# cgrigis/drynx

Hardware: AMD Instinct MI355X
Metric: end-to-end query latency + range-proof verifications/sec, logreg on 1e6 records (higher is better)
Workload: dtype bn254-exact/fp64

## Files before the change

csrc/kernels/dx_gt_t2.hip:

```cpp
#define DX_NI __host__ __device__ __forceinline__
#include "common.h"

namespace {
constexpr int kChunk = 8;

DX_HD bool fp_canonical(const uint32_t *w) {
  uint32_t br = 0;
  for (int k = 0; k < 8; k++) (void)subb32(w[k], FpParams::MOD[k], br);
  return br != 0;
}

DX_HD void compress_chunk(const uint32_t *a, uint32_t *c, uint8_t *ok, int64_t i0, int64_t i1) {
  Fp6 acc = Fp6::one();
  uint32_t good = 0;
  for (int64_t i = i0; i < i1; i++) {
    const uint32_t *w = a + 96 * i;
    bool g = true;
    for (int k = 0; k < 12; k++) g = g && fp_canonical(w + 8 * k);
    const Fp12 f = at<Fp12>(a, i);
    g = g && !(f.c1 == Fp6::zero()) && sub(sqr(f.c0), mul_v(sqr(f.c1))) == Fp6::one();
    at<Fp6>(c, i) = acc;
    if (g) {
      good |= 1u << (i - i0);
      acc = mul(acc, f.c1);
// ... 114 lines not shown
  if (!on_gpu) return kChunk;
  const int64_t c = n / (1024 * 64 * 2);
  return c < 1 ? 1 : (c > kChunk ? kChunk : c);
}

int dx_gt_t2_compress(int on_gpu, void *stream, const uint32_t *a, uint32_t *c, uint8_t *ok, int64_t n) {
  const int64_t k = t2_chunk(on_gpu, n);
  const int64_t chunks = (n + k - 1) / k;
  auto op = [=] __host__ __device__(int64_t t) {
    const int64_t i0 = t * k, i1 = i0 + k < n ? i0 + k : n;
    compress_chunk(a, c, ok, i0, i1);
  };
  return run(on_gpu, stream, chunks, op, true, "gt_t2_compress");
}

int dx_gt_t2_decompress(int on_gpu, void *stream, const uint32_t *c, uint32_t *a, int64_t n) {
  const int64_t k = t2_chunk(on_gpu, n);
  const int64_t chunks = (n + k - 1) / k;
  auto op = [=] __host__ __device__(int64_t t) {
    const int64_t i0 = t * k, i1 = i0 + k < n ? i0 + k : n;
    decompress_chunk(c, a, i0, i1);
  };
  return run(on_gpu, stream, chunks, op, true, "gt_t2_decompress");
}
}
```

csrc/kernels/dx_range.hip:

```cpp
#include "common.h"
#include "../bn254/gt_coop.h"

extern "C" {

int dx_rp_prove_a(int on_gpu, void *stream, const uint32_t *negsB_aff, const uint32_t *V_aff, const uint32_t *t_sc,
                  const uint32_t *gt_table, uint32_t *a_out, int64_t n_items, int S, int L) {
  auto op = [=] __host__ __device__(int64_t it) {
    int64_t j = it % L;
    int64_t p = it / ((int64_t)S * L);
    int64_t pj = p * L + j;
    Fp12 f = final_exp(miller_loop(at<G1A>(negsB_aff, pj), at<G2A>(V_aff, it)));
    Fp12 g = gt_fixed_pow(reinterpret_cast<const Fp12 *>(gt_table), t_sc + 8 * pj);
    at<Fp12>(a_out, it) = mul(f, g);
  };
  return run(on_gpu, stream, n_items, op, true, "rp_prove_a");
}

int dx_rp_prove_a_tab(int on_gpu, void *stream, const uint32_t *gphi_tables, const int32_t *tab_idx,
                      const uint32_t *e_sc, const uint32_t *t_sc, const uint32_t *gt_table, uint32_t *a_out,
                      int64_t n_items, int S, int L, int wbits) {
  const int64_t n_pj = n_items / S;
  auto p1 = [=] __host__ __device__(int64_t pj) {
    const int64_t p = pj / L, j = pj % L;
    at<Fp12>(a_out, p * S * L + j) = gt_fixed_pow(reinterpret_cast<const Fp12 *>(gt_table), t_sc + 8 * pj);
// ... 41 lines not shown
  if (n_slices <= 0) return 0;
  if (!on_gpu) {
    host_for_each(n_slices, [=](int64_t s) {
      const int64_t b = start[s];
      const int n = len[s];
      Fp12 acc = Fp12::one();
      for (int k = 0; k < n; k++) acc = mul(acc, at<Fp12>(src, idx ? idx[b + k] : b + k));
      at<Fp12>(out, s) = acc;
    });
    return 0;
  }
  const unsigned blocks = (unsigned)((n_slices + coop::kTriples - 1) / coop::kTriples);
  hipLaunchKernelGGL(gt_slice_prod_coop, dim3(blocks), dim3(64), 0, (hipStream_t)stream, src, idx, start, len, out,
                     n_slices);
  return check_hip(hipGetLastError(), "gt_slice_prod");
}

namespace {
__global__ void __launch_bounds__(64) DX_OCC gt_chunk_weight_coop(const uint32_t *B, const int32_t *d,
                                                                 const int64_t *start, const int32_t *len,
                                                                 const int32_t *base, uint32_t *out,
                                                                 int64_t n_chunks) {
  const coop::Role R = coop::role();
  const int64_t ch = (int64_t)blockIdx.x * coop::kTriples + R.g;
  if (R.g >= coop::kTriples || ch >= n_chunks) return;
  const Fp12 *F = reinterpret_cast<const Fp12 *>(B);
  const int64_t a = start[ch];
  const int n = len[ch];
  const uint32_t b0 = (uint32_t)base[ch];
  Fp6 acc = coop::one(R), tot = coop::one(R);
// ... 55 lines not shown
```

drynx_amd/native/__init__.py:

```python
from __future__ import annotations

import ctypes
import os
import threading

import numpy as np

import torch

_HERE = os.path.dirname(os.path.abspath(__file__))
LIB_PATH = os.environ.get("DRYNX_NATIVE_LIB") or os.path.join(_HERE, "libdrynx_native.so")

_lib = None


def _load():
    global _lib
    if _lib is not None:
        return _lib
    if not os.path.exists(LIB_PATH):
        if os.environ.get("DRYNX_AUTOBUILD", "1") == "1":
            from . import build as _b

            _b.build()
# ... 107 lines not shown
    "dx_g2_joint_table": [_I, _P, _P, _P, _L],
    "dx_g2_joint_table_signed": [_I, _P, _P, _P, _P, _L],
    "dx_rp_u_group": [_I, _P, _P, _P, _P, _P, _P, _P, _L, _I, _L, _I, _I, _L, _P, _P],
    "dx_rp_u_joint": [_I, _P, _P, _P, _P, _L, _I, _I, _L, _P],
    "dx_g2_slice_sum": [_I, _P, _P, _P, _P, _P, _P, _L, _I, _L],
    "dx_g2_horner": [_I, _P, _P, _P, _I, _I, _I, _L, _L],
    "dx_rp_msm_uv": [_I, _P, _P, _P, _L, _I, _L],
    "dx_msm_keys": [_I, _P, _P, _P, _L, _L, _I, _I, _P, _P],
    "dx_gls8_entries": [],
    "dx_g2_gls8_table": [_I, _P, _P, _P, _P, _L],
    "dx_gt_gls8_table": [_I, _P, _P, _P, _P, _L, _P, _L],
    "dx_g2_gls8_mul": [_I, _P, _P, _P, _P, _P, _L],
    "dx_rp_prove_a_gls8": [_I, _P, _P, _P, _P, _P, _P, _P, _L, _I, _I, _I, _P],
    "dx_gt16_entries": [],
    "dx_gt16_table": [_I, _P, _P, _P, _P],
}


def _declare(lib):
    for name, args in _SIGS.items():
        fn = getattr(lib, name)
        fn.argtypes = args
        fn.restype = ctypes.c_int


def lib():
    return _load()


def loaded_path() -> str:
# ... 145 lines not shown
    _call("dx_g1_fb_mul_i64", g, s, _ptr(table), _ptr(m.contiguous()), _ptr(out), n)
    return out


G1_MUL_PAIR_ROWS = 1 << 14


def gt_t2_compress(a: torch.Tensor, out: torch.Tensor | None = None):
    n = _rows(a, 96)
    c = torch.empty((n, 48), dtype=torch.int32, device=a.device) if out is None else out
    assert c.is_contiguous() and _rows(c, 48) == n
    ok = torch.empty((n,), dtype=torch.uint8, device=a.device)
    g, s = _ctx(a, c)
    _call("dx_gt_t2_compress", g, s, _ptr(a.contiguous()), _ptr(c), _ptr(ok), n)
    return ok if out is not None else (c, ok)


def gt_t2_decompress(c: torch.Tensor, out: torch.Tensor | None = None) -> torch.Tensor:
    n = _rows(c, 48)
    out = torch.empty((n, 96), dtype=torch.int32, device=c.device) if out is None else out
    assert out.is_contiguous() and _rows(out, 96) == n
    g, s = _ctx(c, out)
    _call("dx_gt_t2_decompress", g, s, _ptr(c.contiguous()), _ptr(out), n)
    return out


def g2_x_compress(V: torch.Tensor, x_out: torch.Tensor | None = None, flag_out: torch.Tensor | None = None):
    n = _rows(V, 32)
    x = torch.empty((n, 16), dtype=torch.int32, device=V.device) if x_out is None else x_out
    f = torch.empty((n,), dtype=torch.int32, device=V.device) if flag_out is None else flag_out
# ... 1105 lines not shown
        cur = _gt_prod_level(cur, 8)
    return gt_prod(cur.cpu(), chunk=4).view(1, 96)


def _gt_prod_level(x: torch.Tensor, ch: int) -> torch.Tensor:
    n_items, n_groups = x.shape[0], x.shape[1]
    n_chunks = (n_items + ch - 1) // ch
    out = torch.empty((n_chunks, n_groups, 96), dtype=torch.int32, device=x.device)
    g, s = _ctx(x)
    _call("dx_gt_prod_chunks", g, s, _ptr(x.contiguous()), _ptr(out), n_items, n_groups, ch)
    return out


from .msm import (G2_CHUNK, capture_keep, check_overflow, g1_msm, g1_msm_device, g1_msm_finish,
                  g1_msm_grouped, g1_msm_launch, g1_msm_plan, g1_slice_sum, g2_chunk_weight, g2_msm_device,
                  g2_msm_finish, g2_msm_launch, g2_msm_run, g2_slice_sum, gt_chunk_weight, gt_slice_prod, me_window,
                  multi_exp_device, multi_exp_grouped, multi_exp_grouped_finish, multi_exp_plan, rp_msm_uv)
```

drynx_amd/native/msm.py:

```python
from __future__ import annotations

import threading

import numpy as np

import torch

from . import (_call, _ctx, _gt_prod_level, _pow2_scalar, _ptr, _raw_call, _rows, _upload, g1_mul, gt_mul, gt_one,
               gt_pow, gt_prod)

_ME_SLICE = 8
G2_CHUNK = 32


def gt_slice_prod(src: torch.Tensor, idx, start: torch.Tensor, length: torch.Tensor) -> torch.Tensor:
    n = start.numel()
    out = torch.empty((n, 96), dtype=torch.int32, device=src.device)
    g, s = _ctx(src, idx, start, length)
    _call("dx_gt_slice_prod", g, s, _ptr(src), _ptr(idx), _ptr(start), _ptr(length), _ptr(out), n)
    return out


def g1_slice_sum(src: torch.Tensor, idx, start: torch.Tensor, length: torch.Tensor) -> torch.Tensor:
    n = start.numel()
    out = torch.empty((n, 24), dtype=torch.int32, device=src.device)
    g, s = _ctx(src, idx, start, length)
    _call("dx_g1_slice_sum", g, s, _ptr(src), _ptr(idx), _ptr(start), _ptr(length), _ptr(out), n)
    return out


def g2_slice_sum(src: torch.Tensor, idx, start: torch.Tensor, length: torch.Tensor, src_aff: bool,
                 idx_mod: int = 0) -> torch.Tensor:
    n = start.numel()
    assert src.shape[-1] == (32 if src_aff else 48) and (idx is None or idx.dtype == torch.int32)
# ... 17 lines not shown

def g2_chunk_weight(B_jac: torch.Tensor, d: torch.Tensor, start: torch.Tensor, length: torch.Tensor,
                    base: torch.Tensor) -> torch.Tensor:
    n = start.numel()
    assert B_jac.shape[-1] == 48 and d.dtype == torch.int32 and start.dtype == torch.int64
    assert length.dtype == torch.int32 and base.dtype == torch.int32 and base.numel() == n
    out = torch.empty((n, 48), dtype=torch.int32, device=B_jac.device)
    g, s = _ctx(B_jac, d, start, length, base)
    _call("dx_g2_chunk_weight", g, s, _ptr(B_jac.contiguous()), _ptr(d.contiguous()), _ptr(start), _ptr(length),
          _ptr(base), _ptr(out), n)
    return out


def _gt_ops(a: torch.Tensor, items: torch.Tensor, item_split: tuple | None = None):
    n = a.shape[0]
    it = items.to(torch.int64)
    if item_split is not None:
        sp, q = item_split
        it = torch.where(it < sp, it % n, (it - sp) % q)
    else:
        it = it % n
    it = it.contiguous()
    return (lambda st, ln: gt_slice_prod(a, it, st, ln)), (lambda cur, st, ln: gt_slice_prod(cur, None, st, ln))


def _g1_ops(P_jac: torch.Tensor, items: torch.Tensor):
    P_jac, it = P_jac.contiguous(), items.to(torch.int64)
    return (lambda st, ln: g1_slice_sum(P_jac, it, st, ln)), (lambda cur, st, ln: g1_slice_sum(cur, None, st, ln))


def _g2_ops(P_aff: torch.Tensor, items: torch.Tensor, m: int):
    return (lambda st, ln: g2_slice_sum(P_aff, items, st, ln, True, m)), \
        (lambda cur, st, ln: g2_slice_sum(cur, None, st, ln, False))


def _group_arg(group, n: int, dev):
    if group is None:
        return None, 0
# ... 275 lines not shown
def multi_exp_device(a: torch.Tensor, k: torch.Tensor, group, groups: tuple, W: int | None = None,
                     c: int | None = None, item_split: tuple | None = None) -> dict:
    dev = a.device
    G = len(groups)
    if c is None:
        W, c = me_window(tuple(groups))
    B, lay, overflow = _device_buckets(k, group, groups, W, c, _ME_SLICE, lambda items: _gt_ops(a, items, item_split))
    if "gtw" not in lay:
        lay["gtw"] = _chunk_weight_plan(lay["used"], c, dev)
    wp = lay["gtw"]
    cur = gt_chunk_weight(B, wp["d"], *wp["chunks"])
    for st, ln in wp["gpasses"]:
        cur = gt_slice_prod(cur, None, st, ln)
    win = gt_one(dev).repeat(G * W, 1)
    win.index_copy_(0, wp["gws"], cur)
    return {"G": G, "W": W, "c": c, "win": win.view(1, G * W, 96), "overflow": overflow}


def multi_exp_grouped_finish(h) -> torch.Tensor:
    G, W = h["G"], h["W"]
    if h["win"] is None:
        return gt_one("cpu").repeat(G, 1)
    S_w = gt_prod(h["win"].cpu(), chunk=64).view(G, W, 96)
    acc = S_w[:, W - 1].contiguous()
    sh = _pow2_scalar(h["c"]).expand(G, 8).contiguous()
    for w in range(W - 2, -1, -1):
        acc = gt_mul(gt_pow(acc, sh), S_w[:, w].contiguous())
    return acc


# ... 111 lines not shown
```

drynx_amd/proofs/ledger_codec.py:

```python
from __future__ import annotations

import numpy as np
import torch

from .. import native as nt

MAGIC = 0x32435052
_HEAD = 5
_RW = 5
_GT, _G2 = 0, 1
_FULL = {_GT: 96, _G2: 32}
_SMALL = {_GT: 48, _G2: 17}


def _regions(b, k: int) -> np.ndarray:
    return np.frombuffer(bytes(b[4 * _HEAD: 4 * (_HEAD + _RW * k)]), dtype=np.int32).reshape(k, _RW)


def is_compressed(b) -> bool:
    if len(b) < 4 * _HEAD or len(b) % 4 or int.from_bytes(bytes(b[:4]), "little") != MAGIC:
        return False
    w = np.frombuffer(bytes(b[:4 * _HEAD]), dtype=np.int32)
    k = int(w[4])
    if int(w[1]) != 1 or k < 1 or 4 * (_HEAD + _RW * k) > len(b):
        return False
    total = int(w[2:4].view(np.int64)[0])
    r = _regions(b, k)
    if not np.isin(r[:, 4], (_GT, _G2)).all():
        return False
    m = r[:, 2:4].copy().view(np.int64).reshape(-1)
    saved = sum(int(mi) * (_FULL[int(kd)] - _SMALL[int(kd)]) for mi, kd in zip(m, r[:, 4]))
    return len(b) // 4 == _HEAD + _RW * k + total - saved


class Pending:

    def __init__(self, tensor: torch.Tensor, regions: list | None):
        self.tensor = tensor.contiguous().reshape(-1)
        self.regions = regions
        self.image = None
        self.compact = False

    def produce(self, stream):
        with torch.cuda.stream(stream):
            if self.regions is None:
                self.regions = regions_from_header(self.tensor)
            if not self.regions:
                self.compact = False
                return memoryview(self.tensor.cpu().numpy()).cast("B")
            img = self.launch()
            host = torch.empty((img.numel(),), dtype=torch.uint8, pin_memory=True)
            nt.copy_to_host([(img, host)], host)
            ev = torch.cuda.Event()
            ev.record(stream)
        ev.synchronize()
        return self.finish(memoryview(host.numpy()))

    def launch(self) -> torch.Tensor:
        t = self.tensor
        dev = t.device
        if dev.type == "cuda":
            t.record_stream(torch.cuda.current_stream(dev))
        head = [MAGIC, 0] + list(np.array([t.numel()], dtype=np.int64).view(np.int32)) + [len(self.regions)]
        for off, m, kind in self.regions:
            head += list(np.array([off, m], dtype=np.int64).view(np.int32)) + [kind]
        n_img = len(head) + t.numel() - sum(m * (_FULL[kd] - _SMALL[kd]) for _, m, kd in self.regions)
        img = torch.empty((n_img,), dtype=torch.int32, device=dev)
        hdr = torch.tensor(head, dtype=torch.int32)
        if dev.type == "cuda":
            hdr = hdr.pin_memory().to(dev, non_blocking=True)
        pairs, oks, pos, q = [(hdr, img[:len(head)])], [], 0, len(head)
        for off, m, kind in self.regions:
            pairs.append((t[pos:off], img[q: q + off - pos]))
            q += off - pos
            src = t[off: off + _FULL[kind] * m].view(m, _FULL[kind])
            if kind == _GT:
                oks.append(nt.gt_t2_compress(src, out=img[q: q + 48 * m].view(m, 48)))
            else:
                oks.append(nt.g2_x_compress(src, x_out=img[q: q + 16 * m].view(m, 16),
                                            flag_out=img[q + 16 * m: q + 17 * m])[2])
            q += _SMALL[kind] * m
            pos = off + _FULL[kind] * m
        pairs.append((t[pos:], img[q:]))
        nt.batched_copy(pairs)
        okall = torch.cat(oks).all() if len(oks) > 1 else oks[0].all()
        img[1:2].copy_(okall.to(torch.int32).view(1))
        self.image = img
        return img.view(torch.uint8)

    def finish(self, mv: memoryview):
        self.compact = int.from_bytes(bytes(mv[4:8]), "little") == 1
        if self.compact:
            return mv
        return memoryview(self.tensor.cpu().numpy()).cast("B")


def regions_from_header(t: torch.Tensor) -> list:
    W = t.numel()
    if W < 2:
        return []
    k = int(t[0])
    if k < 1 or 1 + k > W:
        return []
    lens = t[1: 1 + k].cpu().tolist()
    pos, regions = 1 + k, []
    for ln in lens:
        if ln < 5 or pos + ln > W:
            return []
        magic, n, u, l, S = t[pos: pos + 5].cpu().tolist()
# ... 74 lines not shown
```

drynx_amd/proofs/range_proof.py:

```python
from __future__ import annotations

import hashlib
import io
import math
import os
import threading
from dataclasses import dataclass

import numpy as np
import torch

from .. import native as nt
from ..crypto import bn254 as bn
from ..crypto import oracle as O
from ..crypto.elgamal import CipherVector, pk_table
from ..query import PublishSignatureBytes
from ..utils import streams, timers
from ..utils.log import get_logger

log = get_logger("range_proof")

G2_LEN, G1_LEN, GT_LEN, SC_LEN = 128, 64, 384, 32


# ... 292 lines not shown
@dataclass
class RangeProofList:
    u: int
    l: int
    S: int
    offset: list
    cols: list
    commit: CipherVector
    challenge: torch.Tensor = None
    zr: torch.Tensor = None
    D: torch.Tensor = None
    zphi: torch.Tensor = None
    zv: torch.Tensor = None
    V: torch.Tensor = None
    A: torch.Tensor = None

    def __len__(self):
        return len(self.commit)

    @property
    def has_rp(self) -> bool:
        return not (self.u == 0 and self.l == 0)

    def to_bytes(self) -> bytes:
        n = len(self)
        out = io.BytesIO()
        hdr = np.array([n, self.u, self.l, self.S], dtype="<i8")
        out.write(hdr.tobytes())
        out.write(np.asarray(self.offset, dtype="<i8").tobytes())
        out.write(np.asarray(self.cols, dtype="<i8").tobytes())
# ... 74 lines not shown
            o += rows * width
            return v

        commit = CipherVector(take(n, 24), take(n, 24))
        rpl = RangeProofList(u, l, S, offs, cols, commit)
        if rpl.has_rp and n:
            rpl.challenge, rpl.zr, rpl.D = take(n, 8), take(n, 8), take(n, 24)
            rpl.zphi, rpl.zv = take(n * l, 8), take(n * S * l, 8)
            rpl.V, rpl.A = take(n * S * l, 32), take(n * S * l, 96)
        return rpl

    def to(self, device) -> "RangeProofList":
        mv = lambda t: None if t is None else t.to(device)
        return RangeProofList(self.u, self.l, self.S, list(self.offset), list(self.cols), self.commit.to(device),
                              mv(self.challenge), mv(self.zr), mv(self.D), mv(self.zphi), mv(self.zv), mv(self.V),
                              mv(self.A))


def to_base(n: int, b: int, l: int) -> list:
    digits = []
    while n > 0:
        digits.append(n % b)
        n //= b
    while len(digits) < l:
        digits.append(0)
    return digits[:max(l, len(digits))]


def _digits(vals, offs, u: int, l: int) -> np.ndarray:
    try:
        v = np.asarray(vals, dtype=np.int64).reshape(-1)
# ... 364 lines not shown
            msq = _msm_queue(_inputs, r.V, ab_all, G, n, S, l, vstream, segs, table, ygroup=yg)
            for v, uok in zip(vns, msq["u_ok"]):
                v["u_ok"] = uok
        ev_u = torch.cuda.Event()
        ev_u.record(torch.cuda.current_stream(device))
    elif yg is None:
        _inputs()
    with timers.span("rp.verify.passes"), (torch.cuda.stream(aux) if aux is not None else _nullctx()):
        Cp, z = _zcp()
        if not ddirect:
            dpts = torch.cat([Cp.contiguous(), r.D.contiguous()]).repeat(G, 1)
            wc = nt.fr_arith(nt.FR_MUL, w_all, r.challenge)
            dsc = torch.stack([wc.view(G, n, 8), w_all.view(G, n, 8)], 1).reshape(-1, 8).contiguous()
        if aux is None:
            S_R, hR = _pass_r(r.V, r.zphi, rho_all, meta)
        A2, mexp, e_all, dfull = _pass_me(r.A, ab_all, gam_all, rho_all, r.zv, w_all, r.zr, z, meta)
        with timers.span("rp.run.D"):
            if ddirect:
                if cC is None:
                    cC = nt.g1_mul(Cp.contiguous(), r.challenge.contiguous())
                elif ev_cC is not None:
                    torch.cuda.current_stream(device).wait_event(ev_cC)
                pts = torch.stack([cC, r.D], 1).unsqueeze(1).expand(n, G, 2, 24).reshape(-1, 24)
                abs_ = wab_all.view(G, n, 2).permute(1, 0, 2).unsqueeze(2).expand(n, G, 2, 2).reshape(-1, 2)
                dcheck = nt.g1_sum(nt.g1_mul_glv(pts.contiguous(), abs_.contiguous()).view(n, 2 * G, 24))
            else:
                dcheck = nt.g1_msm_device(dpts, dsc, n, ((n, 254),) * (2 * G))
    if aux is None:
        msq = _msm_queue(inp.get("Y", _inputs), r.V, ab_all, G, n, S, l, None, segs, ygroup=yg)
        for v, uok in zip(vns, msq["u_ok"]):
            v["u_ok"] = uok
    useg = fR = None
    with timers.span("rp.verify.multiexp"):
        if aux is not None:
            run_idle_tasks()
            ev_r.synchronize()
            with timers.span("rp.verify.r_tail"):
                fR, rok = _msm_r_miller(hR, S_R)
            ev_u.synchronize()
            with timers.span("rp.verify.u_tail"):
                useg = _seg_products(msq)
            aux.synchronize()
        GG = nt.multi_exp_grouped_finish(mexp)
        D_all = dcheck.cpu() if ddirect else nt.g1_msm_finish(dcheck)
        for h_ in (mexp, hR) if ddirect else (mexp, hR, dcheck):
            nt.check_overflow(h_)
        e_all, dfull = e_all.cpu(), dfull.cpu()
    with timers.span("rp.verify.fold_wait"):
        if useg is None:
            useg = _seg_products(msq)
        for k_, v in enumerate(vns):
            v["F"] = nt.gt_prod(useg[k_].view(-1, 1, 96), chunk=64).view(1, 96)
        if fR is None:
            fR, rok = _msm_r_miller(hR, S_R)
        for v, f, ok in zip(vns, fR, rok):
            v["F"], v["r_ok"] = nt.gt_mul(v["F"], f.view(1, 96)), ok
    for k, v in enumerate(vns):
# ... 107 lines not shown
        t = _SHAPE_INDEX[k] = bn.publish(fn(torch.arange(n, device=device)).contiguous())
    if t.is_cuda:
        t.record_stream(torch.cuda.current_stream(t.device))
    return t


def _pass_r(V, zphi, rho, meta):
    G, m, S, l, gb, wc, cR = meta
    zi = _shape_index(("zphi", m, S, l), V.device,
                      lambda it: (it // (S * l)) * l + it % l, m)
    s_r = nt.fr_arith(nt.FR_MUL, rho, zphi.index_select(0, zi).contiguous())
    with timers.span("rp.run.R"):
        return nt.g2_msm_device(V, s_r, m, ((m, 254),) * G, c=cR)


def _pass_me(A, ab, gam, rho, zv, w, zr, z, meta):
    G, m, S, l, gb, wc, cR = meta
    dev = A.device
    with timers.span("rp.frob8"):
        A2 = torch.empty((2 * m, 96), dtype=torch.int32, device=dev)
        A2[:m].copy_(A)
        nt.gt_frob8(A.contiguous(), out=A2[m:])
    abv = ab.view(G, m, 2)
    k = torch.zeros((3 * G * m, 8), dtype=torch.int32, device=dev)
    kr = k[: 2 * G * m].view(G, 2 * m, 8)
    kr[:, :m, 0] = abv[:, :, 0]
    kr[:, m:, 0] = abv[:, :, 1]
    k[2 * G * m:] = gam
    mgrp = _shape_index(("mgrp", G, m), dev,
                        lambda e: torch.where(e < 2 * G * m, e // (2 * m), G + (e - 2 * G * m) // m).to(torch.int32),
                        3 * G * m)
    with timers.span("rp.run.ME"):
        mexp = nt.multi_exp_device(A2, k, mgrp, ((2 * m, 32),) * G + ((m, gb),) * G, wc[0], wc[1],
                                   item_split=(2 * G * m, m))
    e_all = nt.fr_dot_rows(rho, zv, G, b_periodic=True)
    dfull = torch.stack([nt.fr_dot_rows(w, zr, G, b_periodic=True),
                         nt.fr_dot_rows(w, z, G, b_periodic=True)], 1)
    return A2, mexp, e_all, dfull


_DCHECK_DIRECT_MAX = 16384


def _r_window(m: int, G: int) -> int:
    return min(range(8, 14), key=lambda c: -(-254 // c) * (m + 8 * (1 << c)))


_YGROUP_MIN_MULT = 3
_KEY_GROUPS: dict = {}
# ... 223 lines not shown


def _segment_hinted(r: RangeProofList, segs: list, v: int, T: list, x: dict):
    dev = r.V.device
    n, S, l, G = len(r), r.S, r.l, x["G"]
    m, tot = n * S * l, x["tot"]
    if tot["lhs"][v] is None or tot["dl"][v] is None:
        return None
    poff = np.cumsum([0] + list(segs))
    rT = rpl_cat([rpl_range(r, int(poff[s]), int(poff[s + 1])) for s in T])
    pidx = torch.cat([torch.arange(int(poff[s]), int(poff[s + 1])) for s in T])
    iidx = (pidx.view(-1, 1) * (S * l) + torch.arange(S * l).view(1, -1)).reshape(-1)
    pidx, iidx = bn.h2d(pidx, dev), bn.h2d(iidx, dev)
    sel = lambda t, w, idx: t.view(G, -1, w)[v].index_select(0, idx).contiguous()
    Tt = bn.h2d(torch.tensor(T), x["u_seg"].device)
    xT = dict(A2=x["A2"].index_select(0, torch.cat([iidx, iidx + m])), rho=sel(x["rho"], 8, iidx),
              ab=sel(x["ab"], 2, iidx), gam=sel(x["gam"], 8, iidx), w=sel(x["w"], 8, pidx),
              Cp=x["Cp"].index_select(0, pidx), z=x["z"].index_select(0, pidx),
              useg=x["useg"][v: v + 1, T], u_seg=x["u_seg"][v: v + 1].index_select(1, Tt),
              PB_base=x["PB_base"], gt_tab=x["gt_tab"], wc=x["wc"], G=1, m_first=[x["m_first"][v]])
    comp = {}
    perT = _segment_pass(rT, [segs[s] for s in T], [0], xT, comp)[0]
    if all(perT):
        return None
    inv_lhs = nt.gt_inv(nt.gt_prod(comp["lhs"].view(len(T), 1, 96), chunk=64).view(1, 96))
    lhs_rest = nt.gt_mul(tot["lhs"][v].view(1, 96), inv_lhs)
    e_rest = tot["e"][v: v + 1].cpu()
    for s_ in range(len(T)):
        e_rest = nt.fr_arith(nt.FR_SUB, e_rest, comp["e"][s_: s_ + 1].contiguous())
    eq = bool(nt.gt_eq(lhs_rest, nt.gt_fb_pow(x["gt_tab"], e_rest)).all())
    d1 = nt.g1_sum(torch.cat([tot["dl"][v].view(1, 1, 24), comp["dr"].view(-1, 1, 24)]))
# ... 42 lines not shown
        k[Gf:, :m] = rows(x["gam"], m).view(Gf, m, 8)
    k = k.view(-1, 8)
    fi2 = torch.arange(gam_groups * Gf, device=dev).view(gam_groups * Gf, 1)
    grp2 = (fi2 * nseg + iseg.repeat(2).view(1, 2 * m)).reshape(-1).to(torch.int32)
    wc = nt.fr_arith(nt.FR_MUL, w, r.challenge.contiguous())
    dsc = torch.stack([wc.view(Gf, n, 8), w.view(Gf, n, 8)], 1).reshape(-1, 8).contiguous()
    grp3 = ((fi.view(Gf, 1, 1) * 2 + torch.arange(2, device=dev).view(1, 2, 1)) * nseg
            + pseg.view(1, 1, n)).reshape(-1).to(torch.int32)
    dpts = torch.cat([x["Cp"].contiguous(), r.D.contiguous()]).repeat(Gf, 1)
    with timers.span("rp.seg.plans"):
        hR = nt.g2_msm_launch(r.V, s_r, grp, K, c=_seg_c(Gf * m, K))
        mplan = nt.multi_exp_plan(k, grp2, gam_groups * K, W=x["wc"][0], c=x["wc"][1])
        dplan = nt.g1_msm_plan(dsc, grp3, 2 * K)
    with timers.span("rp.seg.passes"):
        S_R = nt.g2_msm_run(r.V, hR)
        mexp = nt.multi_exp_grouped(x["A2"], k, grp2, gam_groups * K, W=x["wc"][0], c=x["wc"][1], plan=mplan)
        dh = nt.g1_msm_launch(dpts, dsc, grp3, 2 * K, bits=256, plan=dplan)
    offs = torch.from_numpy((np.arange(Gf).reshape(Gf, 1) * n + poff[:-1].reshape(1, nseg)).reshape(-1))
    offs = bn.h2d(torch.cat([offs, torch.tensor([Gf * n])]), dev)
    e = nt.fr_seg_sum(nt.fr_dot_rows(rho, r.zv.repeat(Gf, 1).contiguous(), Gf * n), offs)
    dzr = nt.fr_seg_sum(nt.fr_arith(nt.FR_MUL, w, r.zr.contiguous()), offs)
    dz = nt.fr_seg_sum(nt.fr_arith(nt.FR_MUL, w, x["z"].contiguous()), offs)
    with timers.span("rp.seg.gt_finish"):
        GG = nt.multi_exp_grouped_finish(mexp)
        m_ok = _gt_in_subgroup_each(GG[K:]) if gam_groups == 2 else [True] * K
    if comp is not None and gam_groups == 2:
        comp["GGgam"] = GG[K:].cpu()
    GG = GG[:K]
    with timers.span("rp.seg.r_finish"):
        fR, rok = _msm_r_miller(hR, S_R)
    with timers.span("rp.seg.d_finish"):
# ... 57 lines not shown
    if key not in _aux:
        _aux[key] = torch.cuda.Stream(device, priority=streams.priority(AUX_PRIORITY))
    return _aux[key]


def rpl_cat(lists: list) -> RangeProofList:
    r0 = lists[0]
    if len(lists) == 1:
        return r0
    assert all((r.u, r.l, r.S) == (r0.u, r0.l, r0.S) for r in lists)
    fields = ("challenge", "zr", "D", "zphi", "zv", "V", "A")
    have = [f for f in fields if getattr(r0, f) is not None]
    outs = nt.cat_rows([[r.commit.K for r in lists], [r.commit.C for r in lists]]
                       + [[getattr(r, f) for r in lists] for f in have])
    got = dict(zip(have, outs[2:]))
    return RangeProofList(r0.u, r0.l, r0.S, [o for r in lists for o in r.offset], [c for r in lists for c in r.cols],
                          CipherVector(outs[0], outs[1]), *[got.get(f) for f in fields])


def rpl_range(r: RangeProofList, a: int, b: int) -> RangeProofList:
    l, S = r.l, r.S
    sl = lambda t, w: None if t is None else t[a * w: b * w]
    return RangeProofList(r.u, l, S, r.offset[a:b], r.cols[a:b], r.commit[a:b], sl(r.challenge, 1), sl(r.zr, 1),
                          sl(r.D, 1), sl(r.zphi, l), sl(r.zv, S * l), sl(r.V, S * l), sl(r.A, S * l))


def _slice(r: RangeProofList, k: int) -> RangeProofList:
    l, S = r.l, r.S
    return RangeProofList(r.u, l, S, r.offset[:k], r.cols[:k], r.commit[:k], r.challenge[:k], r.zr[:k], r.D[:k],
                          r.zphi[: k * l], r.zv[: k * S * l], r.V[: k * S * l], r.A[: k * S * l])


# ... 30 lines not shown
```

drynx_amd/protocols/proof_collection.py:

```python
from __future__ import annotations

import json
import os
import time

import torch

from .. import native as nt
from ..ledger import skipchain as skc
from ..parallel.netem import CT_BYTES, POINT_BYTES, SCALAR_BYTES, SIG_BYTES, flow_hops, range_proof_bytes
from .data_collection import all_possible_groups as dcp_groups
from ..parallel.comm import bytes_to_obj, obj_to_bytes
from ..crypto.coins import Coins
from ..proofs import requests as prq
from ..query import query_to_proofs_nbrs
from ..utils import streams, timers
from ..utils.log import get_logger

log = get_logger("proof_collection")


def expected_counts(sq) -> dict:
    q = query_to_proofs_nbrs(sq)
    return dict(zip(prq.QUERY_ORDER, q))
# ... 399 lines not shown
    exp = expected_counts(sq)
    for k in prq.VN_ORDER:
        if counts[k] != exp[k]:
            log.warning(f"{vn.id}: received {counts[k]} {k} proofs, expected {exp[k]}")
    store.update_async(vn.id, f"{sq.SurveyID}/map", json.dumps(bitmap, sort_keys=True).encode())
    ctx.local_bitmaps[(sq.SurveyID, vn.id)] = bitmap
    return bitmap


def start_range_plane(ctx, sq, range_requests: list, staged: bool = False) -> dict:
    import concurrent.futures as cf

    vns = [ctx.cluster.by_id(si.id) for si in sq.Query.RosterVNs.list]
    with timers.timed("RangeFanOut"):
        reqs = fan_out(ctx, sq, range_requests, pool=True)
    second = cf.Future() if staged else None
    out = {"reqs": reqs, "pooled": _pool_async(ctx, sq, reqs, vns, ctx.comm.plane("pool"), second),
           "second_state": second}
    _prefetch_range(ctx, sq, reqs, vns)
    return out


def _prefetch_range(ctx, sq, reqs, vns):
    if any(vn.rank == ctx.rank for vn in vns) and hasattr(ctx, "ledger_values"):
        with timers.span("ledger.prefetch"):
            ctx.ledger_values([r for r in reqs if r.kind == "range" and r.data_digest], range_shape(sq))


def range_stages(ctx, sq) -> int:
    W = ctx.comm.world
    if W <= 1 or os.environ.get("DRYNX_RANGE_STAGES", "0") != "1":
        return 0
    dps, _, _ = _placement(ctx, sq)
    lo, hi = min(dps), max(dps)
    return lo if 0 < lo < hi else 0
# ... 171 lines not shown
```

drynx_amd/services/service.py:

```python
from __future__ import annotations

import copy
import os
import time
from dataclasses import dataclass, field

import torch

from .. import native as nt
from ..crypto.elgamal import CipherVector
from ..ledger.skipchain import SkipBlock
from ..ledger.skipchain import update_chain as skc_update_chain
from ..ops.encoding import cat_proof_batches as dcp_batch_cat
from ..ledger.store import Store
from ..parallel.comm import Comm, LocalComm
from ..parallel.ec_collectives import KeyIndex
from ..parallel.netem import CT_BYTES, POINT_BYTES, flow_hops, tree_edges
from ..parallel.topology import Cluster
from ..proofs import range_proof as rp
from ..proofs import requests as prq
from ..protocols import computing_nodes as cnp
from ..protocols import data_collection as dcp
from ..protocols import proof_collection as pcp
from ..query import PublishSignatureBytes, SurveyQuery, add_diff_p, check_parameters, ivsigs_digest
# ... 141 lines not shown

    def _host_bytes(self, tensors: list):
        from ..ledger.store import Compact
        from ..proofs.ledger_codec import Pending

        items = list(tensors)
        if not any(isinstance(t, Pending) for t in items) and not items[0].is_cuda:
            return lambda: [memoryview(t.numpy()) for t in items]
        if not hasattr(self, "_ledger_stream"):
            self._ledger_stream = torch.cuda.Stream(self.device)
        st = self._ledger_stream
        st.wait_stream(torch.cuda.current_stream(self.device))
        with torch.cuda.stream(st):
            for t in items:
                (t.tensor if isinstance(t, Pending) else t).record_stream(st)
            raw = [t.launch() if isinstance(t, Pending) and t.regions is not None else t for t in items]
            raw = [t for t in raw if not isinstance(t, Pending)]
            sizes = [t.numel() for t in raw]
            host = torch.empty((max(1, sum(sizes)),), dtype=torch.uint8, pin_memory=True)
            pairs, slow, o = [], [], 0
            for t, n in zip(raw, sizes):
                (pairs if n % 4 == 0 and t.data_ptr() % 4 == 0 else slow).append((t, host[o: o + n]))
                o += n
            if pairs:
                nt.copy_to_host(pairs, host)
            for t, h in slow:
                h.copy_(t, non_blocking=True)
            ev = torch.cuda.Event()
            ev.record(st)

        def produce():
# ... 7 lines not shown
                    v = mv[o: o + sizes[k]]
                    v = it.finish(v) if isinstance(it, Pending) else v
                    o += sizes[k]
                    k += 1
                out.append(Compact(v) if isinstance(it, Pending) and it.compact else v)
            return out
        return produce

    def store(self, vn_id: str) -> Store:
        s = self._stores.get(vn_id)
        if s is None or s.closed:
            s = self._stores[vn_id] = Store(os.path.join(self.workdir, f"db_{vn_id}.sqlite"))
        return s

    def run_survey(self, sq: SurveyQuery | None, on_result=None) -> SurveyResult:
        if self.device.type != "cuda":
            return self._run_survey(sq, on_result)
        if not hasattr(self, "_hp_stream"):
            self._hp_stream = torch.cuda.Stream(self.device, priority=streams.priority(-1))
        hp, outer = self._hp_stream, torch.cuda.current_stream(self.device)
        hp.wait_stream(outer)
        with torch.cuda.stream(hp):
            out = self._run_survey(sq, on_result)
        outer.wait_stream(hp)
        return out

    def _run_survey(self, sq: SurveyQuery | None, on_result=None) -> SurveyResult:
        sq = self._broadcast_query(sq)
        self.surveys[sq.SurveyID] = sq
        if sq.Query.Proofs and sq.Query.RosterVNs is not None and sq.SurveyID not in self.vn_surveys:
            self.register_vn_survey(sq)
        if self.rank == 0 and not check_parameters(sq, add_diff_p(sq.Query.DiffP)):
            log.warning("query parameters failed CheckParameters; continuing as the reference does")
        proofs: list = []
        q = sq.Query
        n_groups = len(dcp.all_possible_groups(q.DPDataGen.GroupByValues))
        n_out = q.Operation.NbrOutput
        t_exec = timers.start_timer("JustExecution")
        if self.net is not None:
            self._net_dissemination(sq)
# ... 399 lines not shown
```

Baseline: 386,800.

## Run range-proof multi-exp on torus-compressed GT elements with cached compression images

Range-proof verification now compresses the GT A elements to T2 torus form (Fp6), which halves the data per element. It runs the multi-exponentiation slice products with a torus beta-multiplication kernel, then finishes the window rows back to Fp12. If any live row cannot be compressed, it falls back to the full Fp12 path, and it makes a host sync to check this. Compressed images are cached per payload storage, keyed on the tensor version, and reused by the ledger encoder, so the T2 compression done for ledger bytes is shared with the verifier. This adds global cache state that is cleared at the end of each survey, a host round-trip for the fallback flag, and more complexity.

After: 406,000, median of 4. 4.9% higher.

```diff
diff --git a/csrc/kernels/dx_gt_t2.hip b/csrc/kernels/dx_gt_t2.hip
--- a/csrc/kernels/dx_gt_t2.hip
+++ b/csrc/kernels/dx_gt_t2.hip
@@ -152,6 +152,44 @@
   return run(on_gpu, stream, chunks, op, true, "gt_t2_compress");
 }
 
+int dx_gt_t2_chunk(int on_gpu, int64_t n) { return (int)t2_chunk(on_gpu, n); }
+
+int dx_gt_t2_compress_blocks(int on_gpu, void *stream, const int64_t *desc, int64_t n_blocks, int64_t n_chunks,
+                             int64_t k, uint32_t *c, uint8_t *ok, uint8_t *is_one) {
+  if (n_blocks <= 0 || k < 1 || k > kChunk) return n_blocks <= 0 ? 0 : -1;
+  auto op = [=] __host__ __device__(int64_t t) {
+    int64_t b = 0, hi = n_blocks;
+    while (hi - b > 1) {
+      const int64_t mid = b + (hi - b) / 2;
+      if (desc[4 * mid + 3] <= t) b = mid;
+      else hi = mid;
+    }
+    const int64_t rows = desc[4 * b + 1], off = desc[4 * b + 2];
+    const int64_t i0 = (t - desc[4 * b + 3]) * k, i1 = i0 + k < rows ? i0 + k : rows;
+    if (i0 >= rows) return;
+    const uint32_t *a = reinterpret_cast<const uint32_t *>(desc[4 * b]);
+    compress_chunk(a, c + 48 * off, ok + off, i0, i1);
+    for (int64_t i = i0; i < i1; i++) is_one[off + i] = at<Fp12>(a, i) == Fp12::one() ? 1 : 0;
+  };
+  return run(on_gpu, stream, n_chunks, op, true, "gt_t2_compress_blocks");
+}
+
+int dx_gt_t2_frob8(int on_gpu, void *stream, const uint32_t *ci, uint32_t *co, int64_t n) {
+  struct K3 {
+    Fp2 k[3];
+  } K;
+  {
+    auto p4 = [](const Fp2 &x) { return sqr(sqr(x)); };
+    const Fp2 gi = inv(p4(Fp2::from_limbs(Frob::G2[1])));
+    for (int j = 0; j < 3; j++) K.k[j] = mul(p4(Fp2::from_limbs(Frob::G2[2 * j])), gi);
+  }
+  auto op = [=] __host__ __device__(int64_t i) {
+    const Fp6 b = at<Fp6>(ci, i);
+    at<Fp6>(co, i) = Fp6{mul(b.c0, K.k[0]), mul(b.c1, K.k[1]), mul(b.c2, K.k[2])};
+  };
+  return run(on_gpu, stream, n, op, false, "gt_t2_frob8");
+}
+
 int dx_gt_t2_decompress(int on_gpu, void *stream, const uint32_t *c, uint32_t *a, int64_t n) {
   const int64_t k = t2_chunk(on_gpu, n);
   const int64_t chunks = (n + k - 1) / k;
diff --git a/csrc/kernels/dx_range.hip b/csrc/kernels/dx_range.hip
--- a/csrc/kernels/dx_range.hip
+++ b/csrc/kernels/dx_range.hip
@@ -1,5 +1,6 @@
 #include "common.h"
 #include "../bn254/gt_coop.h"
+#include "../bn254/gt_torus.h"
 
 extern "C" {
 
@@ -79,6 +80,72 @@
   hipLaunchKernelGGL(gt_slice_prod_coop, dim3(blocks), dim3(64), 0, (hipStream_t)stream, src, idx, start, len, out,
                      n_slices);
   return check_hip(hipGetLastError(), "gt_slice_prod");
+}
+
+namespace {
+DX_HD bool beta_marked(const Fp6 &b) {
+  const uint32_t *p = &b.c0.c0.v[0];
+  uint32_t acc = 0;
+  for (int i = 0; i < 48; i++) acc |= p[i];
+  return acc == 0;
+}
+
+__global__ void __launch_bounds__(64) DX_OCC gt_slice_beta_pair(const uint32_t *src, const int64_t *idx,
+                                                               const int64_t *start, const int32_t *len,
+                                                               uint32_t *out, int64_t n_slices) {
+  namespace pr = torus::pair;
+  const pr::Role R = pr::role();
+  const int64_t s = (int64_t)blockIdx.x * pr::kPairs + R.g;
+  if (s >= n_slices) return;
+  const int64_t b = start[s];
+  const int n = len[s];
+  Fp6 x = pr::one(R);
+  int k = 0;
+  for (; k < n; k++) {
+    const Fp6 beta = at<Fp6>(src, idx ? idx[b + k] : b + k);
+    if (beta_marked(beta)) continue;
+    x = pr::sel6(R.r != 0, Fp6::one(), beta);
+    k++;
+    break;
+  }
+  for (; k < n; k++) {
+    const Fp6 beta = at<Fp6>(src, idx ? idx[b + k] : b + k);
+    if (beta_marked(beta)) continue;
+    pr::mul_beta(x, beta, false, R);
+  }
+  pr::store(&at<Fp12>(out, s), x, R);
+}
+}
+
+extern "C" int dx_gt_slice_beta(int on_gpu, void *stream, const uint32_t *src, const int64_t *idx,
+                                const int64_t *start, const int32_t *len, uint32_t *out, int64_t n_slices) {
+  if (n_slices <= 0) return 0;
+  if (!on_gpu) {
+    host_for_each(n_slices, [=](int64_t s) {
+      const int64_t b = start[s];
+      const int n = len[s];
+      Fp12 y = Fp12::one();
+      bool have = false;
+      for (int k = 0; k < n; k++) {
+        const Fp6 beta = at<Fp6>(src, idx ? idx[b + k] : b + k);
+        if (beta_marked(beta)) continue;
+        if (have) torus::mul_beta(y, beta, false);
+        else y = Fp12{beta, Fp6::one()};
+        have = true;
+      }
+      at<Fp12>(out, s) = y;
+    });
+    return 0;
+  }
+  const unsigned blocks = (unsigned)((n_slices + torus::pair::kPairs - 1) / torus::pair::kPairs);
+  hipLaunchKernelGGL(gt_slice_beta_pair, dim3(blocks), dim3(64), 0, (hipStream_t)stream, src, idx, start, len, out,
+                     n_slices);
+  return check_hip(hipGetLastError(), "gt_slice_beta");
+}
+
+extern "C" int dx_gt_finish_rows(int on_gpu, void *stream, uint32_t *a, int64_t n) {
+  auto op = [=] __host__ __device__(int64_t i) { at<Fp12>(a, i) = torus::finish(at<Fp12>(a, i)); };
+  return run(on_gpu, stream, n, op, true, "gt_finish_rows");
 }
 
 namespace {
diff --git a/drynx_amd/native/__init__.py b/drynx_amd/native/__init__.py
--- a/drynx_amd/native/__init__.py
+++ b/drynx_amd/native/__init__.py
@@ -145,6 +145,11 @@
     "dx_rp_prove_a_gls8": [_I, _P, _P, _P, _P, _P, _P, _P, _L, _I, _I, _I, _P],
     "dx_gt16_entries": [],
     "dx_gt16_table": [_I, _P, _P, _P, _P],
+    "dx_gt_t2_chunk": [_I, _L],
+    "dx_gt_t2_compress_blocks": [_I, _P, _P, _L, _L, _L, _P, _P, _P],
+    "dx_gt_t2_frob8": [_I, _P, _P, _P, _L],
+    "dx_gt_slice_beta": [_I, _P, _P, _P, _P, _P, _P, _L],
+    "dx_gt_finish_rows": [_I, _P, _P, _L],
 }
 
 
@@ -320,6 +325,49 @@
     g, s = _ctx(a, c)
     _call("dx_gt_t2_compress", g, s, _ptr(a.contiguous()), _ptr(c), _ptr(ok), n)
     return ok if out is not None else (c, ok)
+
+
+def gt_t2_compress_blocks(blocks: list, out: torch.Tensor | None = None):
+    blocks = list(blocks)
+    dev = blocks[0].device
+    rows = [_rows(b, 96) for b in blocks]
+    n = sum(rows)
+    c = torch.empty((n, 48), dtype=torch.int32, device=dev) if out is None else out
+    assert c.is_contiguous() and _rows(c, 48) == n and c.device == dev
+    ok = torch.empty((n,), dtype=torch.uint8, device=dev)
+    one = torch.empty((n,), dtype=torch.uint8, device=dev)
+    if n == 0:
+        return c, ok, one
+    g, s = _ctx(*blocks)
+    k = int(_raw_call("dx_gt_t2_chunk", g, n))
+    desc = np.empty((len(blocks), 4), dtype=np.int64)
+    off = ch = 0
+    for i, (b, r) in enumerate(zip(blocks, rows)):
+        assert b.is_contiguous()
+        desc[i] = (b.data_ptr(), r, off, ch)
+        off += r
+        ch += -(-r // k)
+    dd = _upload(desc, dev)
+    for b in blocks:
+        _ptr(b)
+    _call("dx_gt_t2_compress_blocks", g, s, _ptr(dd), len(blocks), ch, k, _ptr(c), _ptr(ok), _ptr(one))
+    return c, ok, one
+
+
+def gt_t2_frob8(c: torch.Tensor, out: torch.Tensor | None = None) -> torch.Tensor:
+    n = _rows(c, 48)
+    out = torch.empty((n, 48), dtype=torch.int32, device=c.device) if out is None else out
+    assert out.is_contiguous() and _rows(out, 48) == n
+    g, s = _ctx(c, out)
+    _call("dx_gt_t2_frob8", g, s, _ptr(c.contiguous()), _ptr(out), n)
+    return out
+
+
+def gt_finish_rows(a: torch.Tensor) -> torch.Tensor:
+    assert a.is_contiguous()
+    g, s = _ctx(a)
+    _call("dx_gt_finish_rows", g, s, _ptr(a), _rows(a, 96))
+    return a
 
 
 def gt_t2_decompress(c: torch.Tensor, out: torch.Tensor | None = None) -> torch.Tensor:
@@ -1455,5 +1503,6 @@
 
 from .msm import (G2_CHUNK, capture_keep, check_overflow, g1_msm, g1_msm_device, g1_msm_finish,
                   g1_msm_grouped, g1_msm_launch, g1_msm_plan, g1_slice_sum, g2_chunk_weight, g2_msm_device,
-                  g2_msm_finish, g2_msm_launch, g2_msm_run, g2_slice_sum, gt_chunk_weight, gt_slice_prod, me_window,
+                  g2_msm_finish, g2_msm_launch, g2_msm_run, g2_slice_sum, gt_chunk_weight, gt_slice_beta, gt_slice_prod,
+                  me_window,
                   multi_exp_device, multi_exp_grouped, multi_exp_grouped_finish, multi_exp_plan, rp_msm_uv)
diff --git a/drynx_amd/native/msm.py b/drynx_amd/native/msm.py
--- a/drynx_amd/native/msm.py
+++ b/drynx_amd/native/msm.py
@@ -6,8 +6,8 @@
 
 import torch
 
-from . import (_call, _ctx, _gt_prod_level, _pow2_scalar, _ptr, _raw_call, _rows, _upload, g1_mul, gt_mul, gt_one,
-               gt_pow, gt_prod)
+from . import (_call, _ctx, _gt_prod_level, _pow2_scalar, _ptr, _raw_call, _rows, _upload, g1_mul, gt_finish_rows,
+               gt_mul, gt_one, gt_pow, gt_prod)
 
 _ME_SLICE = 8
 G2_CHUNK = 32
@@ -18,6 +18,14 @@
     out = torch.empty((n, 96), dtype=torch.int32, device=src.device)
     g, s = _ctx(src, idx, start, length)
     _call("dx_gt_slice_prod", g, s, _ptr(src), _ptr(idx), _ptr(start), _ptr(length), _ptr(out), n)
+    return out
+
+
+def gt_slice_beta(src: torch.Tensor, idx, start: torch.Tensor, length: torch.Tensor) -> torch.Tensor:
+    n = start.numel()
+    out = torch.empty((n, 96), dtype=torch.int32, device=src.device)
+    g, s = _ctx(src, idx, start, length)
+    _call("dx_gt_slice_beta", g, s, _ptr(src), _ptr(idx), _ptr(start), _ptr(length), _ptr(out), n)
     return out
 
 
@@ -65,6 +73,7 @@
 
 def _gt_ops(a: torch.Tensor, items: torch.Tensor, item_split: tuple | None = None):
     n = a.shape[0]
+    first = gt_slice_beta if a.shape[-1] == 48 else gt_slice_prod
     it = items.to(torch.int64)
     if item_split is not None:
         sp, q = item_split
@@ -72,7 +81,7 @@
     else:
         it = it % n
     it = it.contiguous()
-    return (lambda st, ln: gt_slice_prod(a, it, st, ln)), (lambda cur, st, ln: gt_slice_prod(cur, None, st, ln))
+    return (lambda st, ln: first(a, it, st, ln)), (lambda cur, st, ln: gt_slice_prod(cur, None, st, ln))
 
 
 def _g1_ops(P_jac: torch.Tensor, items: torch.Tensor):
@@ -378,6 +387,8 @@
         cur = gt_slice_prod(cur, None, st, ln)
     win = gt_one(dev).repeat(G * W, 1)
     win.index_copy_(0, wp["gws"], cur)
+    if a.shape[-1] == 48:
+        gt_finish_rows(win)
     return {"G": G, "W": W, "c": c, "win": win.view(1, G * W, 96), "overflow": overflow}
 
 
diff --git a/drynx_amd/proofs/ledger_codec.py b/drynx_amd/proofs/ledger_codec.py
--- a/drynx_amd/proofs/ledger_codec.py
+++ b/drynx_amd/proofs/ledger_codec.py
@@ -1,4 +1,6 @@
 from __future__ import annotations
+
+import threading
 
 import numpy as np
 import torch
@@ -33,12 +35,99 @@
     return len(b) // 4 == _HEAD + _RW * k + total - saved
 
 
+_IMAGES: dict = {}
+_PAYLOADS: dict = {}
+_IMAGES_LOCK = threading.Lock()
+_IMAGES_MAX = 64
+
+
+class Images:
+    __slots__ = ("c", "ok", "is_one", "event", "stream")
+
+    def __init__(self, c, ok, is_one, event, stream):
+        self.c, self.ok, self.is_one, self.event, self.stream = c, ok, is_one, event, stream
+
+    def wait(self):
+        if self.event is None:
+            return
+        cur = torch.cuda.current_stream(self.c.device)
+        if cur != self.stream:
+            cur.wait_event(self.event)
+            for t in (self.c, self.ok, self.is_one):
+                t.record_stream(cur)
+
+
+def _storage_key(t: torch.Tensor) -> tuple:
+    return str(t.device), t.untyped_storage().data_ptr()
+
+
+def register_payloads(tensors: list):
+    with _IMAGES_LOCK:
+        for t in tensors:
+            if t is not None and t.dtype == torch.int32 and len(_PAYLOADS) < 4 * _IMAGES_MAX:
+                _PAYLOADS.setdefault(_storage_key(t), (t, t._version))
+
+
+def _image_key(b: torch.Tensor):
+    reg = _PAYLOADS.get(_storage_key(b))
+    if reg is None or reg[0]._version != reg[1] or b._version != reg[1]:
+        return None
+    return str(b.device), b.data_ptr(), b.shape[0]
+
+
+def gt_images(blocks: list, out: torch.Tensor | None = None) -> tuple:
+    with _IMAGES_LOCK:
+        keys = [_image_key(b) for b in blocks]
+        got = [None if k is None else _IMAGES.get(k) for k in keys]
+        todo, slot = [], {}
+        where = []
+        for k, b, e in zip(keys, blocks, got):
+            if e is not None:
+                where.append(e)
+            elif k is not None and k in slot:
+                where.append(slot[k])
+            else:
+                if k is not None:
+                    slot[k] = len(todo)
+                where.append(len(todo))
+                todo.append(b)
+        direct = False
+        if todo:
+            direct = out is not None and len(todo) == len(blocks)
+            c, ok, one = nt.gt_t2_compress_blocks(todo, out=out if direct else None)
+            ev = st = None
+            if c.is_cuda:
+                st = torch.cuda.current_stream(c.device)
+                ev = torch.cuda.Event()
+                ev.record(st)
+            fresh, o = [], 0
+            for b in todo:
+                n = b.shape[0]
+                fresh.append(Images(c[o: o + n], ok[o: o + n], one[o: o + n], ev, st))
+                o += n
+            for k, i in slot.items():
+                _IMAGES[k] = fresh[i]
+            while len(_IMAGES) > _IMAGES_MAX:
+                _IMAGES.pop(next(iter(_IMAGES)))
+            where = [fresh[w] if isinstance(w, int) else w for w in where]
+    for e in where:
+        e.wait()
+    return where, direct
+
+
+def drop_images():
+    with _IMAGES_LOCK:
+        _IMAGES.clear()
+        _PAYLOADS.clear()
+
+
 class Pending:
 
     def __init__(self, tensor: torch.Tensor, regions: list | None):
         self.tensor = tensor.contiguous().reshape(-1)
         self.regions = regions
         self.image = None
+        self.images = None
         self.compact = False
 
     def produce(self, stream):
@@ -56,6 +145,10 @@
         ev.synchronize()
         return self.finish(memoryview(host.numpy()))
 
+    def gt_blocks(self) -> list:
+        t = self.tensor
+        return [t[off: off + 96 * m].view(m, 96) for off, m, kind in self.regions or [] if kind == _GT]
+
     def launch(self) -> torch.Tensor:
         t = self.tensor
         dev = t.device
@@ -70,12 +163,15 @@
         if dev.type == "cuda":
             hdr = hdr.pin_memory().to(dev, non_blocking=True)
         pairs, oks, pos, q = [(hdr, img[:len(head)])], [], 0, len(head)
+        gts = iter(self.images if self.images is not None else gt_images(self.gt_blocks())[0])
         for off, m, kind in self.regions:
             pairs.append((t[pos:off], img[q: q + off - pos]))
             q += off - pos
             src = t[off: off + _FULL[kind] * m].view(m, _FULL[kind])
             if kind == _GT:
-                oks.append(nt.gt_t2_compress(src, out=img[q: q + 48 * m].view(m, 48)))
+                e = next(gts)
+                pairs.append((e.c, img[q: q + 48 * m].view(m, 48)))
+                oks.append(e.ok)
             else:
                 oks.append(nt.g2_x_compress(src, x_out=img[q: q + 16 * m].view(m, 16),
                                             flag_out=img[q + 16 * m: q + 17 * m])[2])
@@ -93,6 +189,17 @@
         if self.compact:
             return mv
         return memoryview(self.tensor.cpu().numpy()).cast("B")
+
+
+def launch_many(pendings: list) -> list:
+    blocks = [b for p in pendings for b in p.gt_blocks()]
+    ents = gt_images(blocks)[0] if blocks else []
+    o = 0
+    for p in pendings:
+        n = len(p.gt_blocks())
+        p.images = ents[o: o + n]
+        o += n
+    return [p.launch() for p in pendings]
 
 
 def regions_from_header(t: torch.Tensor) -> list:
diff --git a/drynx_amd/proofs/range_proof.py b/drynx_amd/proofs/range_proof.py
--- a/drynx_amd/proofs/range_proof.py
+++ b/drynx_amd/proofs/range_proof.py
@@ -330,6 +330,7 @@
     zv: torch.Tensor = None
     V: torch.Tensor = None
     A: torch.Tensor = None
+    a_src: list = None
 
     def __len__(self):
         return len(self.commit)
@@ -434,7 +435,7 @@
         mv = lambda t: None if t is None else t.to(device)
         return RangeProofList(self.u, self.l, self.S, list(self.offset), list(self.cols), self.commit.to(device),
                               mv(self.challenge), mv(self.zr), mv(self.D), mv(self.zphi), mv(self.zv), mv(self.V),
-                              mv(self.A))
+                              mv(self.A), None if self.a_src is None else [mv(b) for b in self.a_src])
 
 
 def to_base(n: int, b: int, l: int) -> list:
@@ -829,7 +830,8 @@
             dsc = torch.stack([wc.view(G, n, 8), w_all.view(G, n, 8)], 1).reshape(-1, 8).contiguous()
         if aux is None:
             S_R, hR = _pass_r(r.V, r.zphi, rho_all, meta)
-        A2, mexp, e_all, dfull = _pass_me(r.A, ab_all, gam_all, rho_all, r.zv, w_all, r.zr, z, meta)
+        A2, mexp, e_all, dfull = _pass_me(r.A, ab_all, gam_all, rho_all, r.zv, w_all, r.zr, z, meta, r.a_src,
+                                          mi if masked else None)
         with timers.span("rp.run.D"):
             if ddirect:
                 if cC is None:
@@ -856,6 +858,7 @@
             with timers.span("rp.verify.u_tail"):
                 useg = _seg_products(msq)
             aux.synchronize()
+        mexp = _me_settle(mexp)
         GG = nt.multi_exp_grouped_finish(mexp)
         D_all = dcheck.cpu() if ddirect else nt.g1_msm_finish(dcheck)
         for h_ in (mexp, hR) if ddirect else (mexp, hR, dcheck):
@@ -993,13 +996,80 @@
         return nt.g2_msm_device(V, s_r, m, ((m, 254),) * G, c=cR)
 
 
-def _pass_me(A, ab, gam, rho, zv, w, zr, z, meta):
+class _LazyA2:
+
+    def __init__(self, A):
+        self.A, self.t = A, None
+
+    def __call__(self) -> torch.Tensor:
+        if self.t is None:
+            A = self.A
+            m = A.shape[0]
+            with timers.span("rp.frob8"):
+                A2 = torch.empty((2 * m, 96), dtype=torch.int32, device=A.device)
+                A2[:m].copy_(A)
+                nt.gt_frob8(A.contiguous(), out=A2[m:])
+            self.t = A2
+        return self.t
+
+
+def _a2(x: dict) -> torch.Tensor:
+    a = x["A2"]
+    return a() if isinstance(a, _LazyA2) else a
+
+
+def me_torus() -> bool:
+    return os.environ.get("DRYNX_ME_TORUS", "1") != "0"
+
+
+def _torus_rows(A, a_src, live):
+    from .ledger_codec import gt_images
+
+    m, dev = A.shape[0], A.device
+    blocks = a_src
+    if not blocks or sum(b.shape[0] for b in blocks) != m or not all(
+            b.is_contiguous() and b.dtype == torch.int32 and b.device == dev and b.shape[0] for b in blocks):
+        blocks = [A.contiguous()]
+    B2 = torch.empty((2 * m, 48), dtype=torch.int32, device=dev)
+    ents, direct = gt_images(blocks, out=B2[:m])
+    if not direct:
+        pairs, o = [], 0
+        for e in ents:
+            pairs.append((e.c, B2[o: o + e.c.shape[0]]))
+            o += e.c.shape[0]
+        nt.batched_copy(pairs)
+    ok = torch.cat([e.ok for e in ents]) if len(ents) > 1 else ents[0].ok
+    one = torch.cat([e.is_one for e in ents]) if len(ents) > 1 else ents[0].is_one
+    noimg = (ok == 0) & (one == 0)
+    if live is not None:
+        noimg = noimg & live.reshape(-1).bool()
+    nt.gt_t2_frob8(B2[:m], out=B2[m:])
+    return B2, noimg.any()
+
+
+def _me_settle(mexp: dict) -> dict:
+    fb = mexp.pop("fp12", None)
+    if fb is None:
+        return mexp
+    win = mexp["win"]
+    host = torch.cat([win.reshape(-1), fb[0].to(torch.int32).reshape(1)]).cpu()
+    if int(host[-1]):
+        with timers.span("rp.run.ME_fp12"):
+            return fb[1]()
+    mexp["win"] = host[:-1].view(win.shape)
+    return mexp
+
+
+def _pass_me(A, ab, gam, rho, zv, w, zr, z, meta, a_src=None, live=None):
     G, m, S, l, gb, wc, cR = meta
     dev = A.device
-    with timers.span("rp.frob8"):
-        A2 = torch.empty((2 * m, 96), dtype=torch.int32, device=dev)
-        A2[:m].copy_(A)
-        nt.gt_frob8(A.contiguous(), out=A2[m:])
+    A2 = _LazyA2(A)
+    noimg = None
+    if me_torus():
+        with timers.span("rp.frob8"):
+            src, noimg = _torus_rows(A, a_src, live)
+    else:
+        src = A2()
     abv = ab.view(G, m, 2)
     k = torch.zeros((3 * G * m, 8), dtype=torch.int32, device=dev)
     kr = k[: 2 * G * m].view(G, 2 * m, 8)
@@ -1009,9 +1079,14 @@
     mgrp = _shape_index(("mgrp", G, m), dev,
                         lambda e: torch.where(e < 2 * G * m, e // (2 * m), G + (e - 2 * G * m) // m).to(torch.int32),
                         3 * G * m)
+    def run(rows):
+        return nt.multi_exp_device(rows, k, mgrp, ((2 * m, 32),) * G + ((m, gb),) * G, wc[0], wc[1],
+                                   item_split=(2 * G * m, m))
+
     with timers.span("rp.run.ME"):
-        mexp = nt.multi_exp_device(A2, k, mgrp, ((2 * m, 32),) * G + ((m, gb),) * G, wc[0], wc[1],
-                                   item_split=(2 * G * m, m))
+        mexp = run(src)
+    if noimg is not None:
+        mexp["fp12"] = (noimg, lambda: run(A2()))
     e_all = nt.fr_dot_rows(rho, zv, G, b_periodic=True)
     dfull = torch.stack([nt.fr_dot_rows(w, zr, G, b_periodic=True),
                          nt.fr_dot_rows(w, z, G, b_periodic=True)], 1)
@@ -1265,7 +1340,7 @@
     pidx, iidx = bn.h2d(pidx, dev), bn.h2d(iidx, dev)
     sel = lambda t, w, idx: t.view(G, -1, w)[v].index_select(0, idx).contiguous()
     Tt = bn.h2d(torch.tensor(T), x["u_seg"].device)
-    xT = dict(A2=x["A2"].index_select(0, torch.cat([iidx, iidx + m])), rho=sel(x["rho"], 8, iidx),
+    xT = dict(A2=_a2(x).index_select(0, torch.cat([iidx, iidx + m])), rho=sel(x["rho"], 8, iidx),
               ab=sel(x["ab"], 2, iidx), gam=sel(x["gam"], 8, iidx), w=sel(x["w"], 8, pidx),
               Cp=x["Cp"].index_select(0, pidx), z=x["z"].index_select(0, pidx),
               useg=x["useg"][v: v + 1, T], u_seg=x["u_seg"][v: v + 1].index_select(1, Tt),
@@ -1338,7 +1413,7 @@
         dplan = nt.g1_msm_plan(dsc, grp3, 2 * K)
     with timers.span("rp.seg.passes"):
         S_R = nt.g2_msm_run(r.V, hR)
-        mexp = nt.multi_exp_grouped(x["A2"], k, grp2, gam_groups * K, W=x["wc"][0], c=x["wc"][1], plan=mplan)
+        mexp = nt.multi_exp_grouped(_a2(x), k, grp2, gam_groups * K, W=x["wc"][0], c=x["wc"][1], plan=mplan)
         dh = nt.g1_msm_launch(dpts, dsc, grp3, 2 * K, bits=256, plan=dplan)
     offs = torch.from_numpy((np.arange(Gf).reshape(Gf, 1) * n + poff[:-1].reshape(1, nseg)).reshape(-1))
     offs = bn.h2d(torch.cat([offs, torch.tensor([Gf * n])]), dev)
@@ -1426,8 +1501,9 @@
     outs = nt.cat_rows([[r.commit.K for r in lists], [r.commit.C for r in lists]]
                        + [[getattr(r, f) for r in lists] for f in have])
     got = dict(zip(have, outs[2:]))
+    a_src = [b for r in lists for b in (r.a_src if r.a_src is not None else [r.A])] if r0.A is not None else None
     return RangeProofList(r0.u, r0.l, r0.S, [o for r in lists for o in r.offset], [c for r in lists for c in r.cols],
-                          CipherVector(outs[0], outs[1]), *[got.get(f) for f in fields])
+                          CipherVector(outs[0], outs[1]), *[got.get(f) for f in fields], a_src)
 
 
 def rpl_range(r: RangeProofList, a: int, b: int) -> RangeProofList:
diff --git a/drynx_amd/protocols/proof_collection.py b/drynx_amd/protocols/proof_collection.py
--- a/drynx_amd/protocols/proof_collection.py
+++ b/drynx_amd/protocols/proof_collection.py
@@ -437,11 +437,19 @@
     vns = [ctx.cluster.by_id(si.id) for si in sq.Query.RosterVNs.list]
     with timers.timed("RangeFanOut"):
         reqs = fan_out(ctx, sq, range_requests, pool=True)
+    _register_range_payloads(ctx, reqs, vns)
     second = cf.Future() if staged else None
     out = {"reqs": reqs, "pooled": _pool_async(ctx, sq, reqs, vns, ctx.comm.plane("pool"), second),
            "second_state": second}
     _prefetch_range(ctx, sq, reqs, vns)
     return out
+
+
+def _register_range_payloads(ctx, reqs, vns):
+    if any(vn.rank == ctx.rank for vn in vns) and hasattr(ctx, "ledger_values"):
+        from ..proofs.ledger_codec import register_payloads
+
+        register_payloads([r.tensor for r in reqs if r.kind == "range" and r.tensor is not None and r._data is None])
 
 
 def _prefetch_range(ctx, sq, reqs, vns):
diff --git a/drynx_amd/services/service.py b/drynx_amd/services/service.py
--- a/drynx_amd/services/service.py
+++ b/drynx_amd/services/service.py
@@ -179,7 +179,11 @@
         with torch.cuda.stream(st):
             for t in items:
                 (t.tensor if isinstance(t, Pending) else t).record_stream(st)
-            raw = [t.launch() if isinstance(t, Pending) and t.regions is not None else t for t in items]
+            from ..proofs.ledger_codec import launch_many
+
+            known = [t for t in items if isinstance(t, Pending) and t.regions is not None]
+            built = dict(zip(map(id, known), launch_many(known)))
+            raw = [built.get(id(t), t) for t in items]
             raw = [t for t in raw if not isinstance(t, Pending)]
             sizes = [t.numel() for t in raw]
             host = torch.empty((max(1, sum(sizes)),), dtype=torch.uint8, pin_memory=True)
@@ -217,16 +221,21 @@
         return s
 
     def run_survey(self, sq: SurveyQuery | None, on_result=None) -> SurveyResult:
-        if self.device.type != "cuda":
-            return self._run_survey(sq, on_result)
-        if not hasattr(self, "_hp_stream"):
-            self._hp_stream = torch.cuda.Stream(self.device, priority=streams.priority(-1))
-        hp, outer = self._hp_stream, torch.cuda.current_stream(self.device)
-        hp.wait_stream(outer)
-        with torch.cuda.stream(hp):
-            out = self._run_survey(sq, on_result)
-        outer.wait_stream(hp)
-        return out
+        from ..proofs.ledger_codec import drop_images
+
+        try:
+            if self.device.type != "cuda":
+                return self._run_survey(sq, on_result)
+            if not hasattr(self, "_hp_stream"):
+                self._hp_stream = torch.cuda.Stream(self.device, priority=streams.priority(-1))
+            hp, outer = self._hp_stream, torch.cuda.current_stream(self.device)
+            hp.wait_stream(outer)
+            with torch.cuda.stream(hp):
+                out = self._run_survey(sq, on_result)
+            outer.wait_stream(hp)
+            return out
+        finally:
+            drop_images()
 
     def _run_survey(self, sq: SurveyQuery | None, on_result=None) -> SurveyResult:
         sq = self._broadcast_query(sq)
```
